# osmocom/gr-fosphor

Measured on AMD Instinct MI355X. Metric: complex IQ MSamples/s @1024-pt FFT, higher is better.
Workload: dtype f32

## Files before the change

### gr-fosphor_amd/csrc/fosphor_kernels.hip

```cpp
#include <atomic>

#include "fosphor_internal.h"

#pragma clang fp contract(off)

namespace fosphor_amd {




typedef float v2f __attribute__((ext_vector_type(2)));

#define F_SQRT_1_2 (0.707106781188f)

static __device__ __forceinline__ v2f c_mul(v2f a, v2f w)
{
	v2f t1, t2, r;
	asm("v_pk_mul_f32 %0, %1, %2 op_sel_hi:[1,0]" : "=v"(t1) : "v"(a), "v"(w));
	asm("v_pk_mul_f32 %0, %1, %2 op_sel:[1,1] op_sel_hi:[0,1]" : "=v"(t2) : "v"(a), "v"(w));
	asm("v_pk_add_f32 %0, %1, %2 neg_lo:[0,1]" : "=v"(r) : "v"(t1), "v"(t2));
	return r;
}
template <int N>
static __device__ __forceinline__ void c_mul_n(v2f (&out)[N], const v2f (&in)[N], const v2f (&w)[N])
{
	v2f t1[N], t2[N];
#pragma unroll
	for (int j = 0; j < N; j++)
		asm volatile("v_pk_mul_f32 %0, %1, %2 op_sel_hi:[1,0]" : "=v"(t1[j]) : "v"(in[j]), "v"(w[j]));
#pragma unroll
	for (int j = 0; j < N; j++)
		asm volatile("v_pk_mul_f32 %0, %1, %2 op_sel:[1,1] op_sel_hi:[0,1]" : "=v"(t2[j]) : "v"(in[j]), "v"(w[j]));
#pragma unroll
	for (int j = 0; j < N; j++)
		asm volatile("v_pk_add_f32 %0, %1, %2 neg_lo:[0,1]" : "=v"(out[j]) : "v"(t1[j]), "v"(t2[j]));
}

static __device__ __forceinline__ v2f add_mj(v2f a, v2f b)
{
	v2f r;
	asm("v_pk_add_f32 %0, %1, %2 op_sel:[0,1] op_sel_hi:[1,0] neg_hi:[0,1]" : "=v"(r) : "v"(a), "v"(b));
	return r;
}
static __device__ __forceinline__ v2f sub_mj(v2f a, v2f b)
{
	v2f r;
	asm("v_pk_add_f32 %0, %1, %2 op_sel:[0,1] op_sel_hi:[1,0] neg_lo:[0,1]" : "=v"(r) : "v"(a), "v"(b));
	return r;
}

static __device__ __forceinline__ v2f mul_p1q4(v2f a, v2f s12)
{
	v2f t, r;
	asm("v_pk_add_f32 %0, %1, %1 op_sel:[0,1] op_sel_hi:[1,0] neg_hi:[0,1]" : "=v"(t) : "v"(a));
	asm("v_pk_mul_f32 %0, %1, %2" : "=v"(r) : "v"(t), "v"(s12));
	return r;
}
static __device__ __forceinline__ v2f mul_p3q4(v2f a, v2f s12)
{
	v2f t, r;
	asm("v_pk_add_f32 %0, %1, %1 op_sel:[0,1] op_sel_hi:[0,1] neg_lo:[1,0] neg_hi:[1,1]" : "=v"(t) : "v"(a));
	asm("v_pk_mul_f32 %0, %1, %2" : "=v"(r) : "v"(t), "v"(s12));
	return r;
}

#define DFT2(a, b) do { v2f _t = (a) - (b); (a) = (a) + (b); (b) = _t; } while (0)
#define DFT2_MJ(a, b) do { v2f _t = sub_mj((a), (b)); (a) = add_mj((a), (b)); (b) = _t; } while (0)

static __device__ __forceinline__ void dft8(v2f (&r)[8], v2f s12)
{
	DFT2(r[0], r[4]); DFT2(r[1], r[5]); DFT2(r[2], r[6]); DFT2(r[3], r[7]);
	r[5] = mul_p1q4(r[5], s12); r[7] = mul_p3q4(r[7], s12);
	DFT2(r[0], r[2]); DFT2(r[1], r[3]); DFT2_MJ(r[4], r[6]); DFT2(r[5], r[7]);
	DFT2(r[0], r[1]); DFT2_MJ(r[2], r[3]); DFT2(r[4], r[5]); DFT2_MJ(r[6], r[7]);
}


template <bool SC = false>
static __device__ __forceinline__ void bf(v2f &a, v2f &b, v2f t, v2f two)
{
	v2f u, pa, nb;
	asm("v_pk_fma_f32 %0, %1, %2, %3 op_sel:[1,1,0] op_sel_hi:[0,1,1] neg_lo:[1,0,0]" : "=v"(u) : "v"(b), "v"(t), "v"(a));
	asm("v_pk_fma_f32 %0, %1, %2, %3 op_sel:[0,0,0] op_sel_hi:[1,0,1]" : "=v"(pa) : "v"(b), "v"(t), "v"(u));
	if (SC) asm("v_pk_fma_f32 %0, %1, %2, %3 neg_lo:[0,0,1] neg_hi:[0,0,1]" : "=v"(nb) : "v"(a), "s"(two), "v"(pa));
	else    asm("v_pk_fma_f32 %0, %1, %2, %3 neg_lo:[0,0,1] neg_hi:[0,0,1]" : "=v"(nb) : "v"(a), "v"(two), "v"(pa));
	a = pa; b = nb;
}
template <bool SC = false>
static __device__ __forceinline__ void bf_mj(v2f &a, v2f &b, v2f t, v2f two)
{
	v2f u, pa, nb;
	asm("v_pk_fma_f32 %0, %1, %2, %3 op_sel:[0,1,0] op_sel_hi:[1,1,1]" : "=v"(u) : "v"(b), "v"(t), "v"(a));
	asm("v_pk_fma_f32 %0, %1, %2, %3 op_sel:[1,0,0] op_sel_hi:[0,0,1] neg_hi:[1,0,0]" : "=v"(pa) : "v"(b), "v"(t), "v"(u));
	if (SC) asm("v_pk_fma_f32 %0, %1, %2, %3 neg_lo:[0,0,1] neg_hi:[0,0,1]" : "=v"(nb) : "v"(a), "s"(two), "v"(pa));
	else    asm("v_pk_fma_f32 %0, %1, %2, %3 neg_lo:[0,0,1] neg_hi:[0,0,1]" : "=v"(nb) : "v"(a), "v"(two), "v"(pa));
	a = pa; b = nb;
}
template <bool SC = false>
static __device__ __forceinline__ void bf_s(v2f &a, v2f &b, v2f t, v2f two)
{
	if (!SC) { bf<false>(a, b, t, two); return; }
	v2f u, pa, nb;
	asm("v_pk_fma_f32 %0, %1, %2, %3 op_sel:[1,1,0] op_sel_hi:[0,1,1] neg_lo:[1,0,0]" : "=v"(u) : "v"(b), "s"(t), "v"(a));
	asm("v_pk_fma_f32 %0, %1, %2, %3 op_sel:[0,0,0] op_sel_hi:[1,0,1]" : "=v"(pa) : "v"(b), "s"(t), "v"(u));
	asm("v_pk_fma_f32 %0, %1, %2, %3 neg_lo:[0,0,1] neg_hi:[0,0,1]" : "=v"(nb) : "v"(a), "s"(two), "v"(pa));
	a = pa; b = nb;
}
template <bool SC = false>
static __device__ __forceinline__ void bf_mj_s(v2f &a, v2f &b, v2f t, v2f two)
{
	if (!SC) { bf_mj<false>(a, b, t, two); return; }
	v2f u, pa, nb;
	asm("v_pk_fma_f32 %0, %1, %2, %3 op_sel:[0,1,0] op_sel_hi:[1,1,1]" : "=v"(u) : "v"(b), "s"(t), "v"(a));
	asm("v_pk_fma_f32 %0, %1, %2, %3 op_sel:[1,0,0] op_sel_hi:[0,0,1] neg_hi:[1,0,0]" : "=v"(pa) : "v"(b), "s"(t), "v"(u));
	asm("v_pk_fma_f32 %0, %1, %2, %3 neg_lo:[0,0,1] neg_hi:[0,0,1]" : "=v"(nb) : "v"(a), "s"(two), "v"(pa));
	a = pa; b = nb;
}
template <bool SC, bool TS, int MJ, int I0, int I1, int I2, int I3, int I4, int I5, int I6, int I7, int D, int CNT = 8, bool SW = SC>
static __device__ __forceinline__ void bf8(v2f (&r)[16], v2f t0, v2f t1, v2f t2, v2f t3, v2f t4, v2f t5, v2f t6, v2f t7, v2f two)
{
	constexpr int ia[8] = { I0, I1, I2, I3, I4, I5, I6, I7 };
	const v2f t[8] = { t0, t1, t2, t3, t4, t5, t6, t7 };
	if (SW) {
	v2f u[8], pa[8], nb[8];
#pragma unroll
	for (int j = 0; j < CNT; j++) {
		if (MJ & (1 << j)) {
			if (TS) asm volatile("v_pk_fma_f32 %0, %1, %2, %3 op_sel:[0,1,0] op_sel_hi:[1,1,1]" : "=v"(u[j]) : "v"(r[ia[j] + D]), "s"(t[j]), "v"(r[ia[j]]));
			else    asm volatile("v_pk_fma_f32 %0, %1, %2, %3 op_sel:[0,1,0] op_sel_hi:[1,1,1]" : "=v"(u[j]) : "v"(r[ia[j] + D]), "v"(t[j]), "v"(r[ia[j]]));
		} else {
			if (TS) asm volatile("v_pk_fma_f32 %0, %1, %2, %3 op_sel:[1,1,0] op_sel_hi:[0,1,1] neg_lo:[1,0,0]" : "=v"(u[j]) : "v"(r[ia[j] + D]), "s"(t[j]), "v"(r[ia[j]]));
			else    asm volatile("v_pk_fma_f32 %0, %1, %2, %3 op_sel:[1,1,0] op_sel_hi:[0,1,1] neg_lo:[1,0,0]" : "=v"(u[j]) : "v"(r[ia[j] + D]), "v"(t[j]), "v"(r[ia[j]]));
		}
	}
#pragma unroll
	for (int j = 0; j < CNT; j++) {
		if (MJ & (1 << j)) {
			if (TS) asm volatile("v_pk_fma_f32 %0, %1, %2, %3 op_sel:[1,0,0] op_sel_hi:[0,0,1] neg_hi:[1,0,0]" : "=v"(pa[j]) : "v"(r[ia[j] + D]), "s"(t[j]), "v"(u[j]));
			else    asm volatile("v_pk_fma_f32 %0, %1, %2, %3 op_sel:[1,0,0] op_sel_hi:[0,0,1] neg_hi:[1,0,0]" : "=v"(pa[j]) : "v"(r[ia[j] + D]), "v"(t[j]), "v"(u[j]));
		} else {
			if (TS) asm volatile("v_pk_fma_f32 %0, %1, %2, %3 op_sel:[0,0,0] op_sel_hi:[1,0,1]" : "=v"(pa[j]) : "v"(r[ia[j] + D]), "s"(t[j]), "v"(u[j]));
			else    asm volatile("v_pk_fma_f32 %0, %1, %2, %3 op_sel:[0,0,0] op_sel_hi:[1,0,1]" : "=v"(pa[j]) : "v"(r[ia[j] + D]), "v"(t[j]), "v"(u[j]));
		}
	}
#pragma unroll
	for (int j = 0; j < CNT; j++) {
		if (SC) asm volatile("v_pk_fma_f32 %0, %1, %2, %3 neg_lo:[0,0,1] neg_hi:[0,0,1]" : "=v"(nb[j]) : "v"(r[ia[j]]), "s"(two), "v"(pa[j]));
		else    asm volatile("v_pk_fma_f32 %0, %1, %2, %3 neg_lo:[0,0,1] neg_hi:[0,0,1]" : "=v"(nb[j]) : "v"(r[ia[j]]), "v"(two), "v"(pa[j]));
	}
#pragma unroll
	for (int j = 0; j < CNT; j++) { r[ia[j]] = pa[j]; r[ia[j] + D] = nb[j]; }
	} else {
#pragma unroll
// ... 66 lines not shown
	v2f r; asm("v_pk_mul_f32 %0, %1, %2 op_sel_hi:[1,0]" : "=v"(r) : "v"(x), "v"(w)); return r;
}
static __device__ __forceinline__ v2f mul_bcast_hi(v2f x, v2f w)
{
	v2f r; asm("v_pk_mul_f32 %0, %1, %2 op_sel:[0,1]" : "=v"(r) : "v"(x), "v"(w)); return r;
}

#define R8_PERM(jj) (((jj) == 0) ? 0 : ((jj) == 1) ? 4 : ((jj) == 2) ? 2 : ((jj) == 3) ? 6 : \
                     ((jj) == 4) ? 1 : ((jj) == 5) ? 5 : ((jj) == 6) ? 3 : 7)

static __device__ __forceinline__ void wave_lds_sync()
{
	__builtin_amdgcn_fence(__ATOMIC_RELEASE, "wavefront");
	__builtin_amdgcn_wave_barrier();
	__builtin_amdgcn_fence(__ATOMIC_ACQUIRE, "wavefront");
}


#define F_HALF_LOG10_2 (0.150514997831990597606869447362f)

struct ThrScalar { const double *p; };
typedef uint32_t thr_u4 __attribute__((ext_vector_type(4)));
typedef uint32_t thr_u2 __attribute__((ext_vector_type(2)));
static __device__ __forceinline__ double thr_mk(uint32_t lo, uint32_t hi)
{
	return __longlong_as_double((long long)(((unsigned long long)hi << 32) | lo));
}
template <typename ThrPtr>
static __device__ __forceinline__ void thr_pair(ThrPtr thr, int i, double *t0, double *t1)
{
	*t0 = thr[i];
	*t1 = thr[i + 1];
}
template <>
__device__ __forceinline__ void thr_pair<ThrScalar>(ThrScalar thr, int i, double *t0, double *t1)
{
	double a = 0.0, b = 0.0;
	unsigned long long todo = __builtin_amdgcn_ballot_w64(true);
	while (todo) {
		const int l = __builtin_ctzll(todo);
		const int g = __builtin_amdgcn_readlane(i, l);
		thr_u4 v;
		asm volatile("s_load_dwordx4 %0, %1, 0x0\n\ts_waitcnt lgkmcnt(0)" : "=s"(v) : "s"(thr.p + g) : "memory");
		const bool mine = (i == g);
		if (mine) { a = thr_mk(v.x, v.y); b = thr_mk(v.z, v.w); }
		todo &= ~__builtin_amdgcn_ballot_w64(mine);
	}
	*t0 = a; *t1 = b;
}
template <typename ThrPtr>
static __device__ __forceinline__ double thr_one(ThrPtr thr, int i)
{
	return thr[i];
}
template <>
__device__ __forceinline__ double thr_one<ThrScalar>(ThrScalar thr, int i)
{
	double a = 0.0;
	unsigned long long todo = __builtin_amdgcn_ballot_w64(true);
	while (todo) {
		const int l = __builtin_ctzll(todo);
		const int g = __builtin_amdgcn_readlane(i, l);
		thr_u2 v;
		asm volatile("s_load_dwordx2 %0, %1, 0x0\n\ts_waitcnt lgkmcnt(0)" : "=s"(v) : "s"(thr.p + g) : "memory");
		const bool mine = (i == g);
		if (mine) a = thr_mk(v.x, v.y);
		todo &= ~__builtin_amdgcn_ballot_w64(mine);
	}
	return a;
}

template <typename ThrPtr>
static __device__ __forceinline__ uint32_t bin_exact(float re, float im, float l2_fast, int guess,
                                                      ThrPtr thr, int nb, float *l2_out)
{
	const double xr = (double)re, xi = (double)im;
	const double sd = __builtin_fma(xr, xr, xi * xi);
	const float  sf = (float)sd;
	int bin;

	if (sf >= 1e-30f && sf <= 1e30f) {
		double t0, t1;
		thr_pair(thr, guess, &t0, &t1);
		bin = guess - (sd < t0 ? 1 : 0) + (sd >= t1 ? 1 : 0);
		*l2_out = l2_fast;
	} else {
		int lo = 0, hi = nb;
		const double t_top = thr_one(thr, nb);
		if (sd >= t_top) {
			bin = nb;
		} else if (!(sd >= 0.0)) {
			bin = 0;
		} else {
			while (hi - lo > 1) {
				int mid = (lo + hi) >> 1;
				if (sd >= thr_one(thr, mid)) lo = mid; else hi = mid;
			}
			bin = lo;
		}
		if (__builtin_isinf(re) || __builtin_isinf(im) || sd >= t_top) {
			*l2_out = __builtin_inff();
		} else if (sd == 0.0) {
			*l2_out = -__builtin_inff();
		} else if (sd != sd) {
			*l2_out = __builtin_nanf("");
		} else {
			double sl = sd;
			if (sd < 0x1p-252) {
				const double m = sd * 0x1p298;
				double k = __builtin_rint((double)__builtin_sqrtf((float)m));
				for (int it = 0; it < 2; it++)
					k += (m > __builtin_fma(k, k, k)) ? 1.0 : (m <= __builtin_fma(k, k, -k)) ? -1.0 : 0.0;
				sl = (k * k) * 0x1p-298;
			}
			const unsigned long long u = (unsigned long long)__double_as_longlong(sl);
			const int e = (int)((u >> 52) & 0x7ff) - 1023;
			const double m = __longlong_as_double((long long)((u & 0x000fffffffffffffULL) | 0x3ff0000000000000ULL));
			*l2_out = (float)e + __builtin_amdgcn_logf((float)m);
		}
	}
	if (bin >= nb)
		bin = 0;
	return (uint32_t)bin;
}

struct BinConst { float A, C, amb, kappa; int nb; const double *thr; };

static __device__ __forceinline__ float bin_fast(float re, float im, const BinConst &k, float *l2_out, uint32_t *amb_bits)
{
	const float s  = __builtin_fmaf(re, re, im * im);
	const float l2 = __builtin_amdgcn_logf(s);
	const float v  = __builtin_fmaf(k.A, l2, k.C);
	const float r  = __builtin_rintf(v);
	const float a  = __builtin_fmaf(__builtin_fabsf(l2), k.kappa, __builtin_fabsf(v - r));
	*l2_out = l2;
	*amb_bits = __float_as_uint(a);
	return r;
}

static __device__ __forceinline__ uint32_t pack_bin(float r, float top, uint32_t byte, uint32_t old)
{
	return __builtin_amdgcn_cvt_pk_u8_f32(__builtin_fminf(r, top), byte, old);
}

static __device__ __forceinline__ float max_f32(float a, float b)
{
	float r;
	asm("v_max_f32 %0, %1, %2" : "=v"(r) : "v"(a), "v"(b));
	return r;
}


constexpr int kK1WavesPerSimd = 2;

#ifndef K1_TIMING
#define K1_TIMING 0
#endif
#if K1_TIMING
#define K1_STAMP(i) do { asm volatile("s_waitcnt lgkmcnt(0)" ::: "memory"); \
		const long long _now = __builtin_readcyclecounter(); tacc[i] += _now - tprev; tprev = _now; } while (0)
#else
#define K1_STAMP(i) do { } while (0)
#endif

typedef float v4f __attribute__((ext_vector_type(4)));
typedef uint32_t u2v __attribute__((ext_vector_type(2)));

typedef uint32_t u4v __attribute__((ext_vector_type(4)));
static __device__ __forceinline__ __amdgpu_buffer_rsrc_t make_rsrc(const void *base)
{
	return __builtin_amdgcn_make_buffer_rsrc(const_cast<void *>(base), 0, 0xffffffff, 0x00020000);
}
constexpr int kAuxNT = 2, kAuxSC1 = 16;
template <int AUX>
static __device__ __forceinline__ void bst_v2f(v2f v, __amdgpu_buffer_rsrc_t rs, uint32_t voff, uint32_t soff)
{
	__builtin_amdgcn_raw_buffer_store_b64(u2v{ __float_as_uint(v.x), __float_as_uint(v.y) }, rs, voff, soff, AUX);
}
template <int AUX>
static __device__ __forceinline__ v2f bld_v2f(__amdgpu_buffer_rsrc_t rs, uint32_t voff, uint32_t soff)
{
	const u2v u = __builtin_amdgcn_raw_buffer_load_b64(rs, voff, soff, AUX);
	return v2f{ __uint_as_float(u.x), __uint_as_float(u.y) };
}

constexpr int kIqFp32 = 0, kIqFp16 = 1, kIqSc16 = 2;
static __device__ __forceinline__ v2f widen_sc16(uint32_t v)
{
	return v2f{ (float)(short)(v & 0xffffu) * 0x1p-15f, (float)(short)(v >> 16) * 0x1p-15f };
}
struct iq_fp32 {
	typedef float2 elem;
	static __device__ __forceinline__ v2f ld_sample(const elem *src) { return __builtin_nontemporal_load(reinterpret_cast<const v2f *>(src)); }
	static __device__ __forceinline__ void load_iq16(v2f (&x)[16], const elem *__restrict__ src)
	{
#pragma unroll
		for (int k = 0; k < 8; k++) {
			const v4f q = __builtin_nontemporal_load(reinterpret_cast<const v4f *>(src + 128 * k));
			x[2 * k]     = v2f{ q.x, q.y };
			x[2 * k + 1] = v2f{ q.z, q.w };
		}
	}
	static __device__ __forceinline__ void load_iq8(v2f (&x)[8], const elem *__restrict__ src)
	{
#pragma unroll
		for (int j = 0; j < 8; j++)
			x[j] = __builtin_nontemporal_load(reinterpret_cast<const v2f *>(src + 128 * j));
	}
	typedef v2f raw;
	static __device__ __forceinline__ raw ld_iq(__amdgpu_buffer_rsrc_t rs, uint32_t voff, int j) { return bld_v2f<kAuxNT>(rs, voff, 4096u * (uint32_t)j); }
	static __device__ __forceinline__ void request(raw &d, uint32_t voff, __amdgpu_buffer_rsrc_t rs, int j)
	{
		asm volatile("buffer_load_dwordx2 %0, %1, %2, %3 offen nt" : "=v"(d) : "v"(voff), "s"(rs), "s"(4096u * (uint32_t)j));
	}
	static __device__ __forceinline__ void mov(raw &d, const raw &s) { asm volatile("v_mov_b64 %0, %1" : "=v"(d) : "v"(s)); }
	static __device__ __forceinline__ v2f widen(raw q) { return q; }
};
struct iq_sc16 {
	typedef uint32_t elem;
	static __device__ __forceinline__ v2f ld_sample(const elem *src) { return widen_sc16(__builtin_nontemporal_load(src)); }
	static __device__ __forceinline__ void load_iq16(v2f (&x)[16], const elem *__restrict__ src)
	{
#pragma unroll
		for (int k = 0; k < 8; k++) {
			const u2v q = __builtin_nontemporal_load(reinterpret_cast<const u2v *>(src + 128 * k));
			x[2 * k]     = widen_sc16(q.x);
			x[2 * k + 1] = widen_sc16(q.y);
		}
	}
	static __device__ __forceinline__ void load_iq8(v2f (&x)[8], const elem *__restrict__ src)
	{
#pragma unroll
		for (int j = 0; j < 8; j++)
			x[j] = ld_sample(src + 128 * j);
	}
	typedef uint32_t raw;
	static __device__ __forceinline__ raw ld_iq(__amdgpu_buffer_rsrc_t rs, uint32_t voff, int j) { return __builtin_amdgcn_raw_buffer_load_b32(rs, voff, 2048u * (uint32_t)j, kAuxNT); }
	static __device__ __forceinline__ void request(raw &d, uint32_t voff, __amdgpu_buffer_rsrc_t rs, int j)
	{
		asm volatile("buffer_load_dword %0, %1, %2, %3 offen nt" : "=v"(d) : "v"(voff), "s"(rs), "s"(2048u * (uint32_t)j));
	}
	static __device__ __forceinline__ void mov(raw &d, const raw &s) { asm volatile("v_mov_b32 %0, %1" : "=v"(d) : "v"(s)); }
	static __device__ __forceinline__ v2f widen(raw q) { return widen_sc16(q); }
};
struct iq_fp16 {
	typedef uint32_t elem;
	static __device__ __forceinline__ v2f widen(uint32_t q)
	{
		typedef _Float16 h2 __attribute__((ext_vector_type(2)));
		const h2 h = __builtin_bit_cast(h2, q);
		return v2f{ (float)h.x, (float)h.y };
	}
};
#define K1_LANE_SRC(lane) (2 * (lane))

#include "k1_fft_bin.inc"

__global__ __launch_bounds__(256, kK1WavesPerSimd)
void k1_traffic_twin(const K1Params p)
{
	const int lane   = threadIdx.x & 63;
	const int wv     = threadIdx.x >> 6;
	const int ntiles = p.total / p.tile;
	const int stride = gridDim.x * 4;
	int tile = blockIdx.x * 4 + wv;
	if (tile >= ntiles)
		return;
	v2f xn[16];
	iq_fp32::load_iq16(xn, p.iq + (size_t)tile * p.tile * p.hop + K1_LANE_SRC(lane));
	for (; tile < ntiles; tile += stride) {
		const int t0 = tile * p.tile;
		v2f acc = { 0.0f, 0.0f };
		for (int g0 = 0; g0 < p.tile; g0 += 4) {
#pragma unroll 1
			for (int u = 0; u < 4; u++) {
				const int t = t0 + g0 + u;
				v2f x[16];
#pragma unroll
				for (int m = 0; m < 16; m++)
					x[m] = xn[m];
				const bool last = (g0 + u + 1 == p.tile);
				const int t_next = last ? (tile + stride) * p.tile : t + 1;
				if (!last || tile + stride < ntiles)
					iq_fp32::load_iq16(xn, p.iq + (size_t)t_next * p.hop + K1_LANE_SRC(lane));
#pragma unroll
				for (int m = 0; m < 16; m++)
					acc += x[m];
			}
			uint32_t *dst = p.bins + (size_t)((t0 + g0) >> 2) * kN + lane;
#pragma unroll
			for (int m = 0; m < 16; m++)
				dst[64 * m] = __float_as_uint(acc.x) + (uint32_t)m;
		}
		float2 *pp = p.partial + (size_t)tile * kN + lane;
#pragma unroll
		for (int m = 0; m < 16; m++)
			pp[64 * m] = make_float2(acc.x, acc.y + (float)m);
	}
}

hipError_t launch_k1_traffic_twin(const K1Params &p, hipStream_t s)
{
	const int tiles = p.total / p.tile;
	int blocks = (tiles + 3) / 4;
	if (blocks > kK1MaxBlocks)
		blocks = kK1MaxBlocks;
// ... 66 lines not shown
{
	int dev = 0;
	if (hipGetDevice(&dev) != hipSuccess || dev < 0 || dev >= 64)
		return hipErrorInvalidDevice;
	if (done.load() >> dev & 1)
		return hipSuccess;
	for (int i = 0; i < n; i++) {
		const hipError_t e = hipFuncSetAttribute(reinterpret_cast<const void *>(fns[i]), hipFuncAttributeMaxDynamicSharedMemorySize, lds);
		if (e != hipSuccess)
			return e;
	}
	done.fetch_or(1ull << dev);
	return hipSuccess;
}

template <typename IQ, int NWV>
static hipError_t launch_k1h_form(const K1Params &p0, hipStream_t s)
{
	static const k1_fn fn[2] = { k1h_fused<IQ, false, NWV>, k1h_fused<IQ, true, NWV> };
	constexpr size_t lds = K1hGeom<NWV>::kLds;
	static std::atomic<unsigned long long> attr_dev{0};
	const hipError_t ae = set_lds_once(fn, 2, (int)lds, attr_dev);
	if (ae != hipSuccess)
		return ae;
	hipLaunchKernelGGL(fn[p0.fft_out ? 1 : 0], dim3(256 * 8 / NWV), dim3(64 * NWV), lds, s, p0);
	return hipGetLastError();
}

static hipError_t launch_k1h(const K1Params &p0, hipStream_t s)
{
	if (!p0.sync || !p0.scratch || p0.tile < 4 || p0.tile > 32 || (p0.tile & 3) || p0.total % p0.tile || p0.total / p0.tile >= (1 << 20))
		return hipErrorInvalidValue;
	return p0.iq_format == kIqSc16 ? launch_k1h_form<iq_sc16, 8>(p0, s)
	     : p0.iq_format == kIqFp16 ? launch_k1h_form<iq_fp16, 8>(p0, s) : launch_k1h_form<iq_fp32, 8>(p0, s);
}

static int k1_tile(const K1Shape &s)
{
	const int v = s.tile_knob, total = s.total, batch = s.batch;
	const bool bins16 = s.n_bins > 256 || s.log2n != 10;
	if (v >= (s.log2n == 13 ? 8 : 4) && v <= (s.log2n == 16 ? 32 : 128) && !(v & (v - 1)) && batch % v == 0 && total % v == 0)
		return v;
	if (s.log2n == 16) {
		for (int t = 32; t >= 8; t >>= 1)
			if (batch % t == 0 && total / t >= 32)
				return t;
		return 4;
	}
	if (s.log2n == 13) {
		for (int t = 64; t >= 8; t >>= 1)
			if (batch % t == 0 && total / t >= 256)
				return t;
		return 8;
	}
	if (s.log2n != 10 || bins16) {
		if (total / 16 >= 2048) return 16;
		if (total / 8 >= 2048) return 8;
		return 4;
	}
	for (int t = 64; t >= 8; t >>= 1)
		if (batch % t == 0 && total / t >= 1024)
			return t;
	return 4;
}

static void k1_walk(K1Plan *pl, int cap)
{
	pl->units = pl->tiles < cap ? pl->tiles : cap;
	pl->max_tiles = pl->units > 0 ? (pl->tiles + pl->units - 1) / pl->units : 0;
	pl->min_tiles = pl->units > 0 ? pl->tiles / pl->units : 0;
}

K1Plan k1_plan(const K1Shape &s)
{
	K1Plan pl;
	const bool bins16 = s.n_bins > 256 || s.log2n != 10;
	pl.tile = s.tile > 0 ? s.tile : k1_tile(s);
	pl.tiles = s.total / pl.tile;
	if (s.log2n == 16) {
		pl.kernel = K1_FUSED;
		pl.grid = 256;
		pl.units = 32;
		pl.max_tiles = pl.min_tiles = 0;
		return pl;
	}
	if (bins16 && s.log2n == 10) {
		pl.kernel = K1_BIG;
		k1_walk(&pl, 4096);
		pl.grid = pl.units;
		return pl;
	}
	if (bins16) {
		const int all_cus = s.n_cus > 0 ? s.n_cus : 256;
		pl.kernel = K1_WIDE;
		k1_walk(&pl, (s.share > 0 && s.share < all_cus && pl.tiles % s.share == 0) ? s.share : all_cus);
		pl.grid = pl.units;
		return pl;
	}
	if (s.k1_knob == 2 || (s.hop & 1) || (s.iq_format == kIqSc16 && (s.align & 7))) {
		pl.kernel = K1_V2;
		k1_walk(&pl, 256 * 2 * kK1v2WavesPerSimd);
		pl.grid = pl.units;
		return pl;
	}
	static const int max_blocks = [] { const char *e = getenv("FOSPHOR_AMD_K1_BLOCKS"); const int v = e ? atoi(e) : 0;
	                                   return (v > 0 && v < kK1MaxBlocks) ? v : kK1MaxBlocks; }();
	pl.kernel = K1_WAVE;
	pl.grid = (pl.tiles + 3) / 4;
	if (pl.grid > max_blocks)
		pl.grid = max_blocks;
	k1_walk(&pl, 4 * pl.grid);
	return pl;
}

static K1Plan k1_plan(const K1Params &p)
{
	K1Shape s = {};
	s.log2n = p.log2n; s.n_bins = p.n_bins; s.iq_format = p.iq_format; s.hop = p.hop;
	s.align = (int)((uintptr_t)p.iq & 15);
	s.k1_knob = p.variant == 2 ? 2 : 1;
	s.n_cus = p.n_cus; s.share = p.cus;
	s.total = p.total; s.batch = p.total; s.tile = p.tile;
	return k1_plan(s);
}

template <typename IQ>
static hipError_t launch_k1_as(const K1Params &p, hipStream_t s)
{
	const K1Plan pl = k1_plan(p);
	if (k1_variant_of(pl.kernel) != p.variant)
		return hipErrorInvalidValue;
	if (p.variant == 3) {
		if (p.log2n == 10) {
			constexpr int N = 1024;
			constexpr int lds = (N + ((N / 2 - 8) / 7) * 7 + N / 2) * 8 + N * 4;
			hipLaunchKernelGGL((p.fft_out ? k1big_fft_bin<IQ, 10, true> : k1big_fft_bin<IQ, 10, false>), dim3(pl.grid), dim3(N / 8), lds, s, p);
			return hipGetLastError();
		}
		if (p.log2n != 13 || (p.tile & 7) || (p.total & 7))
			return hipErrorInvalidValue;
		constexpr int ldsw = 2 * 8192 * 8 + 520 * 8;
		static const k1_fn fns[5] = { k1w_fft_bin<IQ, 8>, k1w_fft_bin<IQ, 4>, k1w_fft_bin<IQ, 2>, k1w_fft_bin<IQ, 1>, k1w_fft_bin<IQ, 16> };
		static std::atomic<unsigned long long> attr_dev{0};
		const hipError_t ae = set_lds_once(fns, 5, ldsw, attr_dev);
		if (ae != hipSuccess)
			return ae;
		const int which = (p.hop == 4096) ? 0 : (p.hop == 2048) ? 1 : (p.hop == 1024) ? 2 : (p.hop == 512) ? 3 : 4;
		hipLaunchKernelGGL(fns[which], dim3(pl.grid), dim3(512), ldsw, s, p);
		return hipGetLastError();
	}
	if (p.variant == 2) {
		hipLaunchKernelGGL((p.fft_out ? k1v2_fft_bin<IQ, true> : k1v2_fft_bin<IQ, false>), dim3(pl.grid), dim3(128), 0, s, p);
		return hipGetLastError();
	}
	hipLaunchKernelGGL((p.fft_out ? k1_fft_bin<IQ, true, false> : p.n_bins == 256 ? k1_fft_bin<IQ, false, true> : k1_fft_bin<IQ, false, false>),
	                   dim3(pl.grid), dim3(256), 0, s, p);
	return hipGetLastError();
}

hipError_t launch_k1(const K1Params &p, hipStream_t s)
{
	if (p.variant == 4)
		return launch_k1h(p, s);
	if (p.iq_format == kIqFp32)
		return launch_k1_as<iq_fp32>(p, s);
	if (p.iq_format == kIqSc16)
		return launch_k1_as<iq_sc16>(p, s);
	return hipErrorInvalidValue;
}

__global__ __launch_bounds__(256)
void k_bin_hook(const float2 *__restrict__ fft, uint8_t *__restrict__ bin, float *__restrict__ pwr, int n,
                const K1Params p, int force_exact)
{
	const BinConst bk = { p.binA, p.binC, p.amb, p.kappa, p.n_bins, p.thr };
	const float top = (float)(bk.nb - 1);
	for (int i = blockIdx.x * blockDim.x + threadIdx.x; i < n; i += gridDim.x * blockDim.x) {
		float2 v = fft[i];
		float l2; uint32_t ab;
		const float r = bin_fast(v.x, v.y, bk, &l2, &ab);
		uint32_t b = p.bins16 ? (uint32_t)(int)__builtin_amdgcn_fmed3f(r, 0.0f, top) : (pack_bin(r, top, 0, 0) & 0xff);
		if (ab > __float_as_uint(bk.amb) || force_exact)
			b = bin_exact(v.x, v.y, l2, (int)__builtin_amdgcn_fmed3f(r, 0.0f, top), ThrScalar{ bk.thr }, bk.nb, &l2);
		if (p.bins16)
			reinterpret_cast<uint16_t *>(bin)[i] = (uint16_t)b;
		else
			bin[i] = (uint8_t)b;
		pwr[i] = l2 * F_HALF_LOG10_2;
	}
}

hipError_t launch_bin_hook(const float2 *fft, uint8_t *bin, float *pwr, int n,
                           const K1Params &p, int force_exact, hipStream_t s)
{
	int blocks = (n + 255) / 256;
	if (blocks > 4096) blocks = 4096;
	hipLaunchKernelGGL(k_bin_hook, dim3(blocks), dim3(256), 0, s, fft, bin, pwr, n, p, force_exact);
	return hipGetLastError();
}


#ifdef K2_TIMING
__device__ unsigned long long g_k2_time[16];
#define K2_STAMP(i) do { if (tid == 0) { const long long _n = __builtin_readcyclecounter(); atomicAdd(&g_k2_time[i], (unsigned long long)(_n - k2prev)); k2prev = _n; } } while (0)
#else
#define K2_STAMP(i) do { } while (0)
#endif
static __device__ __forceinline__ void lds_count(uint32_t *h, uint32_t bin, uint32_t hc4, uint32_t inc)
{
	atomicAdd(reinterpret_cast<uint32_t *>(reinterpret_cast<char *>(h) + ((bin << 7) + hc4)), inc);
}
static __device__ __forceinline__ uint32_t lo16(uint32_t v) { uint32_t r; asm("v_and_b32 %0, 0xffff, %1" : "=v"(r) : "v"(v)); return r; }
static __device__ __forceinline__ uint32_t lo8(uint32_t v)  { uint32_t r; asm("v_and_b32 %0, 0xff, %1" : "=v"(r) : "v"(v)); return r; }

template <int NW, int IF>
__global__ __launch_bounds__(64 * NW)
void k2_count(const K2Params p)
{
	extern __shared__ __attribute__((aligned(16))) uint32_t h[];
	__shared__ float red_s[NW][64], red_m[NW][64];

	const int tid  = threadIdx.x;
	const int lane = tid & 63;
	const int wv   = __builtin_amdgcn_readfirstlane(tid >> 6);
	const int x0   = blockIdx.x * 64;
	const int c    = blockIdx.y;
	const int cpb  = p.batch / p.chunk;
	const int f    = c / cpb;
	const int t_in = (c - f * cpb) * p.chunk;
	const int nb   = p.n_bins;
	const int hcol = lane & 31;
	const uint32_t inc = (lane & 32) ? 0x10000u : 1u;
#ifdef K2_TIMING
	long long k2prev = __builtin_readcyclecounter();
	if (tid == 0) atomicAdd(&g_k2_time[15], 1ull);
#endif

	__shared__ uint32_t rowbits[16];
	{
		uint4 *h4 = reinterpret_cast<uint4 *>(h);
		for (int i = tid; i < nb * 8; i += 64 * NW)
			h4[i] = make_uint4(0u, 0u, 0u, 0u);
	}
	if (tid < 16)
		rowbits[tid] = 0;
	K2_STAMP(0);
	__syncthreads();
	K2_STAMP(1);

	if (p.bins9) {
		const uint32_t n = p.n, qpt = (uint32_t)p.tile >> 2, ntl = (uint32_t)(p.chunk / p.tile);
		const uint32_t *lo = p.bins + (size_t)c * (p.chunk >> 2) * n + x0 + lane;
		const uint32_t *hi = p.bins + (size_t)(p.total >> 2) * n + (size_t)c * ntl * n + x0 + lane;
#pragma unroll 1
		for (uint32_t tl = wv; tl < ntl; tl += NW) {
			const uint32_t hv = __builtin_nontemporal_load(&hi[(size_t)tl * n]);
			uint32_t v[8];
#pragma unroll
			for (uint32_t u = 0; u < 8; u++)
				v[u] = (u < qpt) ? __builtin_nontemporal_load(&lo[(size_t)(tl * qpt + u) * n]) : 0u;
#pragma unroll
			for (uint32_t u = 0; u < 8; u++) {
				if (u < qpt) {
					const uint32_t h4 = hv >> (4 * u);
					atomicAdd(&h[(((v[u]      ) & 0xff) | ((h4 & 1u) << 8)) * 32 + hcol], inc);
					atomicAdd(&h[(((v[u] >>  8) & 0xff) | ((h4 & 2u) << 7)) * 32 + hcol], inc);
					atomicAdd(&h[(((v[u] >> 16) & 0xff) | ((h4 & 4u) << 6)) * 32 + hcol], inc);
					atomicAdd(&h[(((v[u] >> 24)       ) | ((h4 & 8u) << 5)) * 32 + hcol], inc);
				}
			}
		}
	} else if (p.bins8p1) {
		const __amdgpu_buffer_rsrc_t rlo = make_rsrc(reinterpret_cast<const char *>(p.bins) + ((size_t)c * (p.chunk >> 1) * p.n + x0) * 2);
		const __amdgpu_buffer_rsrc_t rhi = make_rsrc(reinterpret_cast<const char *>(p.bins) + (size_t)p.total * p.n + (size_t)c * (p.chunk >> 3) * p.n + x0);
		const uint32_t noct = (uint32_t)p.chunk >> 3, rowlo = 2u * (uint32_t)p.n, rowhi = (uint32_t)p.n;
		const uint32_t lane2 = 2u * (uint32_t)lane, hc4 = 4u * (uint32_t)hcol;
		auto count8 = [&](uint32_t hv, const uint32_t (&v)[4]) {
#pragma unroll
			for (int u = 0; u < 4; u++) {
				lds_count(h, lo8(v[u]) | ((hv << (8 - 2 * u)) & 0x100u), hc4, inc);
				lds_count(h, ((v[u] >> 8) & 0xffu) | ((hv << (7 - 2 * u)) & 0x100u), hc4, inc);
			}
		};
		uint32_t o = wv;
#pragma unroll 1
		for (; o + NW < noct; o += 2 * NW) {
			const uint32_t so_l = (uint32_t)__builtin_amdgcn_readfirstlane((int)(o * 4u * rowlo));
			const uint32_t so_h = (uint32_t)__builtin_amdgcn_readfirstlane((int)(o * rowhi));
			uint32_t va[4], vb[4];
			const uint32_t ha = __builtin_amdgcn_raw_buffer_load_b8(rhi, (uint32_t)lane, so_h, 0);
			const uint32_t hb = __builtin_amdgcn_raw_buffer_load_b8(rhi, (uint32_t)lane, so_h + (uint32_t)NW * rowhi, 0);
#pragma unroll
			for (int u = 0; u < 4; u++) {
				va[u] = __builtin_amdgcn_raw_buffer_load_b16(rlo, lane2, so_l + (uint32_t)u * rowlo, 0);
				vb[u] = __builtin_amdgcn_raw_buffer_load_b16(rlo, lane2, so_l + (uint32_t)(4 * NW + u) * rowlo, 0);
			}
			count8(ha, va);
			count8(hb, vb);
		}
#pragma unroll 1
		for (; o < noct; o += NW) {
			const uint32_t so_l = (uint32_t)__builtin_amdgcn_readfirstlane((int)(o * 4u * rowlo));
			uint32_t va[4];
			const uint32_t ha = __builtin_amdgcn_raw_buffer_load_b8(rhi, (uint32_t)lane, (uint32_t)__builtin_amdgcn_readfirstlane((int)(o * rowhi)), 0);
#pragma unroll
			for (int u = 0; u < 4; u++)
// ... 738 lines not shown
```

### gr-fosphor_amd/csrc/k1_fft_bin.inc

```
template <typename IQ, bool WRITE_FFT, bool NB256 = false>
__global__ __launch_bounds__(256, kK1WavesPerSimd)
void k1_fft_bin(const K1Params p)
{
	__shared__ v2f   lds[4][kN];
	__shared__ v2f   tw4_tab[512];
	__shared__ float win_tab[kN];
	__shared__ double thr_tab[264];

	const int lane   = threadIdx.x & 63;
	const int wv     = __builtin_amdgcn_readfirstlane(threadIdx.x >> 6);
	const int ntiles = p.total / p.tile;
	const int stride = gridDim.x * 4;
#if K1_TIMING
	const long long t_wave_start = wall_clock64();
#endif
	int tile = blockIdx.x * 4 + wv;
	const v2f *twg = reinterpret_cast<const v2f *>(p.tw);
	const typename IQ::elem *iq = reinterpret_cast<const typename IQ::elem *>(p.iq);

	for (int i = threadIdx.x; i < kN; i += 256)
		win_tab[i] = p.win[i];
	for (int i = threadIdx.x; i < 512; i += 256)
		tw4_tab[i] = twg[kTw4Off + i];
	for (int i = threadIdx.x; i <= p.n_bins && i < 264; i += 256)
		thr_tab[i] = p.thr[i];
	__syncthreads();

	if (tile >= ntiles)
		return;

	v2f *buf = lds[wv];

	v2f tw2[7];
	v2f tw3[7];
#pragma unroll
	for (int n = 0; n < 7; n++) {
		tw2[n] = twg[kTw2Off + (lane & 7) * 7 + n];
		tw3[n] = twg[kTw3Off + lane * 7 + n];
	}
	const v2f s12 = { F_SQRT_1_2, F_SQRT_1_2 };

	const int rd_even = lane ^ ((lane >> 3) & 7);
	const int rd_odd  = rd_even ^ 8;
	const int st1     = (8 * lane) ^ (lane & 15);
	const int st1a    = (16 * lane) ^ ((2 * lane) & 15);
	const int st1b    = (16 * lane + 8) ^ ((2 * lane + 1) & 15);
	(void)st1; (void)st1a; (void)st1b;
	const int st2     = ((64 * (lane >> 3)) + (lane & 7)) ^ (lane & 8);

	const BinConst bk = { p.binA, p.binC, p.amb, p.kappa, p.n_bins, p.thr };
	const float vmax_init = -1000.0f / F_HALF_LOG10_2;

	v2f xn[16];
	IQ::load_iq16(xn, iq + (size_t)tile * p.tile * p.hop + K1_LANE_SRC(lane));
#if K1_TIMING
	long long tacc[8] = {0, 0, 0, 0, 0, 0, 0, 0};
	long long tprev = __builtin_readcyclecounter();
#endif

	for (; tile < ntiles; tile += stride) {
	const int t0 = tile * p.tile;

	float live[16], vmax[16];
#pragma unroll
	for (int m = 0; m < 16; m++) {
		live[m] = 0.0f;
		vmax[m] = vmax_init;
	}

	uint32_t pack[16];
#pragma unroll
	for (int m = 0; m < 16; m++)
		pack[m] = 0;
	int pend_row = -1;
	auto flush_pack = [&]() {
		uint32_t *dst = p.bins + (size_t)pend_row * kN + lane;
#pragma unroll
		for (int m = 0; m < 16; m++)
			dst[64 * m] = pack[m];
#pragma unroll
		for (int m = 0; m < 16; m++)
			pack[m] = 0;
		pend_row = -1;
	};

	for (int g0 = 0; g0 < p.tile; g0 += 4) {
#pragma unroll 1
		for (int u = 0; u < 4; u++) {
			const int t = t0 + g0 + u;
			v2f x[16];

			K1_STAMP(7);
#pragma unroll
			for (int k = 0; k < 8; k++) {
				const v2f w = *reinterpret_cast<const v2f *>(&win_tab[2 * lane + 128 * k]);
				x[2 * k]     = mul_bcast_lo(xn[2 * k], w);
				x[2 * k + 1] = mul_bcast_hi(xn[2 * k + 1], w);
			}

			if (u == 0 && pend_row >= 0)
				flush_pack();
			{
				const bool last = (g0 + u + 1 == p.tile);
				const int t_next = last ? (tile + stride) * p.tile : t + 1;
				if (!last || tile + stride < ntiles)
					IQ::load_iq16(xn, iq + (size_t)t_next * p.hop + K1_LANE_SRC(lane));
			}

			K1_STAMP(0);
#pragma unroll
			for (int v = 0; v < 2; v++) {
				v2f r[8];
#pragma unroll
				for (int j = 0; j < 8; j++)
					r[j] = x[v + 2 * j];
				dft8(r, s12);
#pragma unroll
				for (int jj = 0; jj < 8; jj++)
					buf[(v ? st1b : st1a) ^ jj] = r[R8_PERM(jj)];
			}
			wave_lds_sync();
#pragma unroll
			for (int m = 0; m < 16; m++)
				x[m] = buf[((m & 1) ? rd_odd : rd_even) + 64 * m];
			wave_lds_sync();

			K1_STAMP(1);
#pragma unroll
			for (int v = 0; v < 2; v++) {
				v2f r[8];
				{
					v2f in7[7], out7[7];
#pragma unroll
					for (int j = 1; j < 8; j++)
						in7[j - 1] = x[v + 2 * j];
					c_mul_n<7>(out7, in7, tw2);
					r[0] = x[v];
#pragma unroll
					for (int j = 1; j < 8; j++)
						r[j] = out7[j - 1];
				}
				dft8(r, s12);
#pragma unroll
				for (int jj = 0; jj < 8; jj++)
					buf[(st2 ^ (9 * jj)) + 512 * v] = r[R8_PERM(jj)];
			}
			wave_lds_sync();
#pragma unroll
			for (int m = 0; m < 16; m++)
				x[m] = buf[((m & 1) ? rd_odd : rd_even) + 64 * m];
			wave_lds_sync();

			K1_STAMP(2);
			{
				v2f y[16];
#pragma unroll
				for (int v = 0; v < 2; v++) {
					v2f r[8];
					{
						v2f in7[7], out7[7];
#pragma unroll
						for (int j = 1; j < 8; j++)
							in7[j - 1] = x[v + 2 * j];
						c_mul_n<7>(out7, in7, tw3);
						r[0] = x[v];
#pragma unroll
						for (int j = 1; j < 8; j++)
							r[j] = out7[j - 1];
					}
					dft8(r, s12);
#pragma unroll
					for (int jj = 0; jj < 8; jj++)
						y[jj + 8 * v] = r[R8_PERM(jj)];
				}
#pragma unroll
				for (int m = 0; m < 16; m++)
					x[m] = y[m];
			}

			K1_STAMP(3);
			{
				v2f in8[8], w8[8], out8[8];
#pragma unroll
				for (int c = 0; c < 8; c++) { in8[c] = x[c + 8]; w8[c] = tw4_tab[lane + 64 * c]; }
				c_mul_n<8>(out8, in8, w8);
#pragma unroll
				for (int c = 0; c < 8; c++) {
					v2f a = x[c];
					v2f b = out8[c];
					DFT2(a, b);
					x[c] = a;
					x[c + 8] = b;
				}
			}

			K1_STAMP(4);
			if (WRITE_FFT) {
#pragma unroll
				for (int m = 0; m < 16; m++)
					reinterpret_cast<v2f *>(p.fft_out)[(size_t)t * kN + lane + 64 * m] = x[m];
			}

			float    l2[16];
			uint32_t amb = 0;
			const float top = (float)(bk.nb - 1);
#pragma unroll
			for (int m = 0; m < 16; m++) {
				uint32_t ab;
				const float r = bin_fast(x[m].x, x[m].y, bk, &l2[m], &ab);
				amb = amb > ab ? amb : ab;
				pack[m] = NB256 ? __builtin_amdgcn_cvt_pk_u8_f32(r, (uint32_t)u, pack[m]) : pack_bin(r, top, (uint32_t)u, pack[m]);
			}
			if (amb > __float_as_uint(bk.amb)) {
#pragma unroll
				for (int m = 0; m < 16; m++) {
					const float v = __builtin_fmaf(bk.A, l2[m], bk.C);
					const float r = __builtin_rintf(v);
					const float a = __builtin_fmaf(__builtin_fabsf(l2[m]), bk.kappa, __builtin_fabsf(v - r));
					if (!(a <= bk.amb)) {
						const int guess = (int)__builtin_amdgcn_fmed3f(r, 0.0f, top);
						float nl2;
						const uint32_t nbn = bin_exact(x[m].x, x[m].y, l2[m], guess,
						                               (const __attribute__((address_space(3))) double *)thr_tab, bk.nb, &nl2);
						pack[m] = (pack[m] & ~(0xffu << (8 * u))) | (nbn << (8 * u));
						l2[m] = nl2;
					}
				}
			}

#pragma unroll
			for (int m = 0; m < 16; m++) {
				asm("v_fma_f32 %0, %0, %1, %2" : "+v"(live[m]) : "s"(p.w), "v"(l2[m]));
				vmax[m] = max_f32(vmax[m], l2[m]);
			}
			if (t >= p.wf_first) {
				float *wf_row = p.wf + (size_t)((p.wf_pos0 + t) & p.wf_mask) * kN + lane;
#pragma unroll
				for (int m = 0; m < 16; m++)
					wf_row[64 * m] = l2[m] * F_HALF_LOG10_2;
			}
			K1_STAMP(6);
		}

		K1_STAMP(5);
		pend_row = (t0 + g0) >> 2;
	}
	if (pend_row >= 0)
		flush_pack();

	float2 *pp = p.partial + (size_t)tile * kN + lane;
#pragma unroll
	for (int m = 0; m < 16; m++)
		pp[64 * m] = make_float2(live[m] * F_HALF_LOG10_2,
		                         (vmax[m] == vmax_init) ? -1000.0f : vmax[m] * F_HALF_LOG10_2);
	}
#if K1_TIMING
	if (p.dbg && lane == 0) {
		const int w = blockIdx.x * 4 + wv;
		for (int i = 0; i < 8; i++)
			p.dbg[w * 8 + i] = tacc[i];
		p.dbg[w * 8 + 3] = t_wave_start;
		p.dbg[w * 8 + 5] = wall_clock64();
	}
#endif
}
```

Baseline: 552,500.

## Prefetch IQ via global_load_lds DMA and defer accumulate/waterfall tail

Adds an fp32-IQ path that prefetches the next frame's samples straight into LDS with global_load_lds_dwordx4, replacing the register prefetch of 16 complex values. The windowing step now reads those samples from LDS. In mode 2 it also holds each frame's log-power results and runs the accumulate/max/waterfall-store tail for the previous frame between the FFT stages. The aim is to cut VGPR pressure and hide global-load and store latency behind FFT work. In exchange it relies on hand-written m0 handling, vmcnt bookkeeping and the reuse of the per-wave LDS buffer, which makes ordering errors easy.

```diff
diff --git a/gr-fosphor_amd/csrc/fosphor_kernels.hip b/gr-fosphor_amd/csrc/fosphor_kernels.hip
--- a/gr-fosphor_amd/csrc/fosphor_kernels.hip
+++ b/gr-fosphor_amd/csrc/fosphor_kernels.hip
@@ -1,4 +1,5 @@
 #include <atomic>
+#include <type_traits>
 
 #include "fosphor_internal.h"
 
@@ -371,6 +372,10 @@
 
 
 constexpr int kK1WavesPerSimd = 2;
+#ifndef K1_DMA
+#define K1_DMA 2
+#endif
+constexpr int kK1Dma = K1_DMA;
 
 #ifndef K1_TIMING
 #define K1_TIMING 0
@@ -743,6 +748,13 @@
 	if (p.variant == 2) {
 		hipLaunchKernelGGL((p.fft_out ? k1v2_fft_bin<IQ, true> : k1v2_fft_bin<IQ, false>), dim3(pl.grid), dim3(128), 0, s, p);
 		return hipGetLastError();
+	}
+	if constexpr (std::is_same<IQ, iq_fp32>::value && kK1Dma != 0) {
+		if (!p.fft_out && ((uintptr_t)p.iq & 15) == 0) {
+			hipLaunchKernelGGL((p.n_bins == 256 ? k1_fft_bin<IQ, false, true, kK1Dma> : k1_fft_bin<IQ, false, false, kK1Dma>),
+			                   dim3(pl.grid), dim3(256), 0, s, p);
+			return hipGetLastError();
+		}
 	}
 	hipLaunchKernelGGL((p.fft_out ? k1_fft_bin<IQ, true, false> : p.n_bins == 256 ? k1_fft_bin<IQ, false, true> : k1_fft_bin<IQ, false, false>),
 	                   dim3(pl.grid), dim3(256), 0, s, p);
diff --git a/gr-fosphor_amd/csrc/k1_fft_bin.inc b/gr-fosphor_amd/csrc/k1_fft_bin.inc
--- a/gr-fosphor_amd/csrc/k1_fft_bin.inc
+++ b/gr-fosphor_amd/csrc/k1_fft_bin.inc
@@ -1,8 +1,8 @@
-template <typename IQ, bool WRITE_FFT, bool NB256 = false>
+template <typename IQ, bool WRITE_FFT, bool NB256 = false, int DMA = 0>
 __global__ __launch_bounds__(256, kK1WavesPerSimd)
 void k1_fft_bin(const K1Params p)
 {
-	__shared__ v2f   lds[4][kN];
+	__shared__ __attribute__((aligned(16))) v2f lds[4][kN];
 	__shared__ v2f   tw4_tab[512];
 	__shared__ float win_tab[kN];
 	__shared__ double thr_tab[264];
@@ -51,8 +51,37 @@
 	const BinConst bk = { p.binA, p.binC, p.amb, p.kappa, p.n_bins, p.thr };
 	const float vmax_init = -1000.0f / F_HALF_LOG10_2;
 
+	const uint32_t dma_vo = 16u * (unsigned)lane;
+	const uint32_t buf_lds = (uint32_t)(size_t)(__attribute__((address_space(3))) void *)buf;
+	auto request_iq = [&](const typename IQ::elem *src) {
+		uint32_t keep;
+		asm volatile("s_waitcnt lgkmcnt(0)\n\ts_mov_b32 %0, m0\n\ts_mov_b32 m0, %2\n\ts_nop 0\n\t"
+		             "global_load_lds_dwordx4 %1, %3 nt\n\ts_add_u32 m0, m0, 0x400\n\ts_nop 0\n\t"
+		             "global_load_lds_dwordx4 %1, %4 nt\n\ts_add_u32 m0, m0, 0x400\n\ts_nop 0\n\t"
+		             "global_load_lds_dwordx4 %1, %5 nt\n\ts_add_u32 m0, m0, 0x400\n\ts_nop 0\n\t"
+		             "global_load_lds_dwordx4 %1, %6 nt\n\ts_add_u32 m0, m0, 0x400\n\ts_nop 0\n\t"
+		             "global_load_lds_dwordx4 %1, %7 nt\n\ts_add_u32 m0, m0, 0x400\n\ts_nop 0\n\t"
+		             "global_load_lds_dwordx4 %1, %8 nt\n\ts_add_u32 m0, m0, 0x400\n\ts_nop 0\n\t"
+		             "global_load_lds_dwordx4 %1, %9 nt\n\ts_add_u32 m0, m0, 0x400\n\ts_nop 0\n\t"
+		             "global_load_lds_dwordx4 %1, %10 nt\n\ts_mov_b32 m0, %0"
+		             : "=&s"(keep) : "v"(dma_vo), "s"(buf_lds), "s"(src), "s"(src + 128), "s"(src + 256), "s"(src + 384),
+		               "s"(src + 512), "s"(src + 640), "s"(src + 768), "s"(src + 896) : "memory", "scc");
+	};
+	auto iq_wait = [&](int n) {
+		if (n == 16)      asm volatile("s_waitcnt vmcnt(16)" ::: "memory");
+		else if (n == 32) asm volatile("s_waitcnt vmcnt(32)" ::: "memory");
+		else if (n == 48) asm volatile("s_waitcnt vmcnt(48)" ::: "memory");
+		else              asm volatile("s_waitcnt vmcnt(0)" ::: "memory");
+	};
+	int behind = 0;
+
 	v2f xn[16];
-	IQ::load_iq16(xn, iq + (size_t)tile * p.tile * p.hop + K1_LANE_SRC(lane));
+	if constexpr (DMA) {
+		static_assert(sizeof(typename IQ::elem) == 8 && !WRITE_FFT, "the LDS-DMA forms: fp32 IQ, no FFT hook");
+		request_iq(iq + (size_t)tile * p.tile * p.hop);
+	} else {
+		IQ::load_iq16(xn, iq + (size_t)tile * p.tile * p.hop + K1_LANE_SRC(lane));
+	}
 #if K1_TIMING
 	long long tacc[8] = {0, 0, 0, 0, 0, 0, 0, 0};
 	long long tprev = __builtin_readcyclecounter();
@@ -73,6 +102,21 @@
 	for (int m = 0; m < 16; m++)
 		pack[m] = 0;
 	int pend_row = -1;
+	float l2h[16];
+	int held_t = -1;
+	auto tail = [&](auto lo, auto hi) {
+#pragma unroll
+		for (int m = lo; m < hi; m++) {
+			asm("v_fma_f32 %0, %0, %1, %2" : "+v"(live[m]) : "s"(p.w), "v"(l2h[m]));
+			vmax[m] = max_f32(vmax[m], l2h[m]);
+		}
+		if (held_t >= p.wf_first) {
+			float *wf_row = p.wf + (size_t)((p.wf_pos0 + held_t) & p.wf_mask) * kN + lane;
+#pragma unroll
+			for (int m = lo; m < hi; m++)
+				wf_row[64 * m] = l2h[m] * F_HALF_LOG10_2;
+		}
+	};
 	auto flush_pack = [&]() {
 		uint32_t *dst = p.bins + (size_t)pend_row * kN + lane;
 #pragma unroll
@@ -90,17 +134,37 @@
 			const int t = t0 + g0 + u;
 			v2f x[16];
 
+			if constexpr (DMA) {
+				iq_wait(behind);
+				behind = 0;
+			}
 			K1_STAMP(7);
+			if constexpr (DMA) {
+				v4f q[8];
+				v2f w[8];
+#pragma unroll
+				for (int k = 0; k < 8; k++) {
+					q[k] = reinterpret_cast<const v4f *>(buf)[64 * k + lane];
+					w[k] = *reinterpret_cast<const v2f *>(&win_tab[2 * lane + 128 * k]);
+				}
+				asm volatile("s_waitcnt lgkmcnt(0)" ::: "memory");
+#pragma unroll
+				for (int k = 0; k < 8; k++) {
+					x[2 * k]     = mul_bcast_lo(v2f{ q[k].x, q[k].y }, w[k]);
+					x[2 * k + 1] = mul_bcast_hi(v2f{ q[k].z, q[k].w }, w[k]);
+				}
+			} else {
 #pragma unroll
 			for (int k = 0; k < 8; k++) {
 				const v2f w = *reinterpret_cast<const v2f *>(&win_tab[2 * lane + 128 * k]);
 				x[2 * k]     = mul_bcast_lo(xn[2 * k], w);
 				x[2 * k + 1] = mul_bcast_hi(xn[2 * k + 1], w);
 			}
+			}
 
 			if (u == 0 && pend_row >= 0)
 				flush_pack();
-			{
+			if constexpr (!DMA) {
 				const bool last = (g0 + u + 1 == p.tile);
 				const int t_next = last ? (tile + stride) * p.tile : t + 1;
 				if (!last || tile + stride < ntiles)
@@ -119,6 +183,10 @@
 				for (int jj = 0; jj < 8; jj++)
 					buf[(v ? st1b : st1a) ^ jj] = r[R8_PERM(jj)];
 			}
+			if constexpr (DMA == 2) {
+				if (held_t >= 0)
+					tail(std::integral_constant<int, 0>(), std::integral_constant<int, 8>());
+			}
 			wave_lds_sync();
 #pragma unroll
 			for (int m = 0; m < 16; m++)
@@ -145,11 +213,21 @@
 				for (int jj = 0; jj < 8; jj++)
 					buf[(st2 ^ (9 * jj)) + 512 * v] = r[R8_PERM(jj)];
 			}
+			if constexpr (DMA == 2) {
+				if (held_t >= 0)
+					tail(std::integral_constant<int, 8>(), std::integral_constant<int, 16>());
+			}
 			wave_lds_sync();
 #pragma unroll
 			for (int m = 0; m < 16; m++)
 				x[m] = buf[((m & 1) ? rd_odd : rd_even) + 64 * m];
 			wave_lds_sync();
+			if constexpr (DMA) {
+				const bool last = (g0 + u + 1 == p.tile);
+				const int t_next = last ? (tile + stride) * p.tile : t + 1;
+				if (!last || tile + stride < ntiles)
+					request_iq(iq + (size_t)t_next * p.hop);
+			}
 
 			K1_STAMP(2);
 			{
@@ -228,6 +306,12 @@
 				}
 			}
 
+			if constexpr (DMA == 2) {
+#pragma unroll
+				for (int m = 0; m < 16; m++)
+					l2h[m] = l2[m];
+				held_t = t;
+			} else {
 #pragma unroll
 			for (int m = 0; m < 16; m++) {
 				asm("v_fma_f32 %0, %0, %1, %2" : "+v"(live[m]) : "s"(p.w), "v"(l2[m]));
@@ -238,6 +322,9 @@
 #pragma unroll
 				for (int m = 0; m < 16; m++)
 					wf_row[64 * m] = l2[m] * F_HALF_LOG10_2;
+				if constexpr (DMA == 1)
+					behind += 16;
+			}
 			}
 			K1_STAMP(6);
 		}
@@ -245,8 +332,18 @@
 		K1_STAMP(5);
 		pend_row = (t0 + g0) >> 2;
 	}
-	if (pend_row >= 0)
+	if constexpr (DMA == 2) {
+		if (held_t >= 0) {
+			behind += (held_t >= p.wf_first) ? 16 : 0;
+			tail(std::integral_constant<int, 0>(), std::integral_constant<int, 16>());
+			held_t = -1;
+		}
+	}
+	if (pend_row >= 0) {
 		flush_pack();
+		behind += 16;
+	}
+	behind += 16;
 
 	float2 *pp = p.partial + (size_t)tile * kN + lane;
 #pragma unroll
```

Result: slower. 535,900 (-3.0%).
